# SHI-Labs/Self-Similarity-Grouping

Measured on AMD Instinct MI355X. Metric: images/s embed + s/iter for NxN rerank+DBSCAN, N=16k, 1/2/4/8 GPU, higher is better.
Workload: dtype f32 (embed: split-half operands hi+lo on fp16 MFMA, fp32 accumulate, 6e-8 max error vs the fp32 reference features) / exact int64 via int8 MFMA digits + f64 + f16 (distance, re-rank: half semantics, bit-exact)

## Files before the change

self-similarity-grouping_amd/csrc/conv.hip:

```cpp
#include "ssg_common.h"
#include <cstdlib>
#include <type_traits>

namespace ssg {

typedef float v16f __attribute__((ext_vector_type(16)));
typedef unsigned int v4u __attribute__((ext_vector_type(4)));
typedef _Float16 v8h __attribute__((ext_vector_type(8)));

__device__ __forceinline__ unsigned pack_h2(_Float16 a, _Float16 b) {
  return (unsigned)__builtin_bit_cast(unsigned short, a) | ((unsigned)__builtin_bit_cast(unsigned short, b) << 16);
}
__device__ __forceinline__ float unpack_lo(unsigned u) { return (float)__builtin_bit_cast(_Float16, (unsigned short)(u & 0xffffu)); }
__device__ __forceinline__ float unpack_hi(unsigned u) { return (float)__builtin_bit_cast(_Float16, (unsigned short)(u >> 16)); }
__device__ __forceinline__ void split_encode4(const float4 v, uint2& hi, uint2& lo) {
  const _Float16 h0 = (_Float16)v.x, h1 = (_Float16)v.y, h2 = (_Float16)v.z, h3 = (_Float16)v.w;
  hi = make_uint2(pack_h2(h0, h1), pack_h2(h2, h3));
  lo = make_uint2(pack_h2((_Float16)(v.x - (float)h0), (_Float16)(v.y - (float)h1)), pack_h2((_Float16)(v.z - (float)h2), (_Float16)(v.w - (float)h3)));
}
__device__ __forceinline__ bool split_hi_nonfinite(const uint2 hi) {
  const unsigned a = hi.x & 0x7fff7fffu, b = hi.y & 0x7fff7fffu;
  return (a & 0xffffu) >= 0x7c00u || (a >> 16) >= 0x7c00u || (b & 0xffffu) >= 0x7c00u || (b >> 16) >= 0x7c00u;
}
__device__ __forceinline__ float4 split_decode4(const uint2 hi, const uint2 lo) {
// ... 776 lines not shown
            const unsigned a0 = rr[it][0], a1 = rr[it][1], a2 = rr[it][2], a3 = rr[it][3];
            if (n + 1 < NP) rr[it] = __builtin_amdgcn_raw_buffer_load_b128(res_rsrc, poff(n + 1, it), 0, SSG_DMA_RES_AUX);
            const unsigned g0 = lane_xor1(odd ? a0 : a2), g1 = lane_xor1(odd ? a1 : a3);
            const float4 r4 = split_decode4(make_uint2(odd ? g0 : a0, odd ? g1 : a1), make_uint2(odd ? a2 : g0, odd ? a3 : g1));
            v.x += r4.x; v.y += r4.y; v.z += r4.z; v.w += r4.w;
          }
          v.x = v.x > 0.f ? v.x : 0.f; v.y = v.y > 0.f ? v.y : 0.f; v.z = v.z > 0.f ? v.z : 0.f; v.w = v.w > 0.f ? v.w : 0.f;
          uint2 hp, lp;
          split_encode4(v, hp, lp);
          ovf |= ((hp.x & 0x7c007c00u) + 0x04000400u) | ((hp.y & 0x7c007c00u) + 0x04000400u);
          const unsigned rx = lane_xor1(odd ? hp.x : lp.x), ry = lane_xor1(odd ? hp.y : lp.y);
          const v4u stv = {odd ? rx : hp.x, odd ? ry : hp.y, odd ? lp.x : rx, odd ? lp.y : ry};
          __builtin_amdgcn_raw_buffer_store_b128(stv, out_rsrc, poff(n, it), 0, RES ? SSG_DMA_OUT_AUX_RES : SSG_DMA_OUT_AUX);
        }
        __builtin_amdgcn_fence(__ATOMIC_ACQ_REL, "wavefront");
        if (n % MT == MT - 1) { bias = bias_n; cs = cs_n; }
      }
    };
    if (resp) run(std::true_type{}); else run(std::false_type{});
    if ((ovf & 0x80008000u) && p.overflow) *p.overflow = 1;
    SSG_DMA_STAMP(4)
    return;
  }
#pragma unroll
  for (int i = 0; i < MT; i++) {
    const int mbase = tm * BM + wm * WM + i * 32;
#pragma unroll
    for (int j = 0; j < NT; j++) {
      const int col = tn * BN + wn * WN + j * 32 + chunk * 4;
      const float4 bias = *reinterpret_cast<const float4*>(p.bias + col);
      const float4 cs = p.cscale ? *reinterpret_cast<const float4*>(p.cscale + col) : make_float4(1.f, 1.f, 1.f, 1.f);
      float4 rr[ITS];
      if (resp) {
#pragma unroll
        for (int it = 0; it < ITS; it++) {
          const int m = mbase + it * RPI + prow;
          rr[it] = *reinterpret_cast<const float4*>(resp + (int64_t)(m < p.M ? m : 0) * p.Cout + col);
        }
      }
#pragma unroll
      for (int q = 0; q < 4; q++)
        *reinterpret_cast<float4*>(patch + l32 * EP + 8 * q + 4 * h) = make_float4(acc[i][j][4 * q], acc[i][j][4 * q + 1], acc[i][j][4 * q + 2], acc[i][j][4 * q + 3]);
      __builtin_amdgcn_fence(__ATOMIC_ACQ_REL, "wavefront");
#pragma unroll
      for (int it = 0; it < ITS; it++) {
        const int m = mbase + it * RPI + prow;
        float4 v = *reinterpret_cast<const float4*>(patch + (it * RPI + prow) * EP + chunk * 4);
        v.x = v.x * cs.x + bias.x; v.y = v.y * cs.y + bias.y; v.z = v.z * cs.z + bias.z; v.w = v.w * cs.w + bias.w;
        if (resp) {
          float4 r4 = rr[it];
          if (p.res_split) {
            const unsigned s0 = odd ? __float_as_uint(r4.x) : __float_as_uint(r4.z), s1 = odd ? __float_as_uint(r4.y) : __float_as_uint(r4.w);
            const unsigned g0 = lane_xor1(s0), g1 = lane_xor1(s1);
            r4 = odd ? split_decode4(make_uint2(g0, g1), make_uint2(__float_as_uint(r4.z), __float_as_uint(r4.w)))
                     : split_decode4(make_uint2(__float_as_uint(r4.x), __float_as_uint(r4.y)), make_uint2(g0, g1));
          }
          v.x += r4.x; v.y += r4.y; v.z += r4.z; v.w += r4.w;
        }
        if (p.relu) { v.x = v.x > 0.f ? v.x : 0.f; v.y = v.y > 0.f ? v.y : 0.f; v.z = v.z > 0.f ? v.z : 0.f; v.w = v.w > 0.f ? v.w : 0.f; }
        if (p.out_split) {
          uint2 hp, lp;
          split_encode4(v, hp, lp);
          if (p.overflow && split_hi_nonfinite(hp)) *p.overflow = 1;
          const uint2 send = odd ? hp : lp;
          const uint2 recv = make_uint2(lane_xor1(send.x), lane_xor1(send.y));
          const uint4 stv = odd ? make_uint4(recv.x, recv.y, lp.x, lp.y) : make_uint4(hp.x, hp.y, recv.x, recv.y);
          if (m < p.M) *reinterpret_cast<uint4*>(outp + (int64_t)m * p.Cout + col) = stv;
        } else if (m < p.M) *reinterpret_cast<float4*>(outp + (int64_t)m * p.Cout + col) = v;
      }
      __builtin_amdgcn_fence(__ATOMIC_ACQ_REL, "wavefront");
    }
  }
}

__global__ void nchw_to_nhwc4_kernel(const float* __restrict__ in, float* __restrict__ out, int B, int H, int W, int flip) {
  const int64_t total = (int64_t)B * H * W;
  for (int64_t x = (int64_t)blockIdx.x * blockDim.x + threadIdx.x; x < total; x += (int64_t)gridDim.x * blockDim.x) {
    const int w = (int)(x % W); const int64_t t = x / W; const int hh = (int)(t % H); const int b = (int)(t / H);
    const int ws = flip ? (W - 1 - w) : w;
    const int64_t plane = (int64_t)H * W, base = (int64_t)b * 3 * plane + (int64_t)hh * W + ws;
    reinterpret_cast<float4*>(out)[x] = make_float4(in[base], in[base + plane], in[base + 2 * plane], 0.f);
  }
}

__global__ void nchw_to_nhwc4_h4l4_kernel(const float* __restrict__ in, float* __restrict__ out, int B, int H, int W, int flip) {
  const int64_t total = (int64_t)B * H * W;
  for (int64_t x = (int64_t)blockIdx.x * blockDim.x + threadIdx.x; x < total; x += (int64_t)gridDim.x * blockDim.x) {
    const int w = (int)(x % W); const int64_t t = x / W; const int hh = (int)(t % H); const int b = (int)(t / H);
    const int ws = flip ? (W - 1 - w) : w;
    const int64_t plane = (int64_t)H * W, base = (int64_t)b * 3 * plane + (int64_t)hh * W + ws;
    uint2 hi, lo;
    split_encode4(make_float4(in[base], in[base + plane], in[base + 2 * plane], 0.f), hi, lo);
    reinterpret_cast<uint4*>(out)[x] = make_uint4(hi.x, hi.y, lo.x, lo.y);
  }
}

__global__ void maxpool3x3s2_kernel(const float* __restrict__ in, float* __restrict__ out, int B, int H, int W, int C, int OH, int OW) {
  const int C4 = C / 4;
  const int64_t total = (int64_t)B * OH * OW * C4;
  for (int64_t x = (int64_t)blockIdx.x * blockDim.x + threadIdx.x; x < total; x += (int64_t)gridDim.x * blockDim.x) {
    const int c4 = (int)(x % C4); int64_t t = x / C4;
    const int ow = (int)(t % OW); t /= OW; const int oh = (int)(t % OH); const int b = (int)(t / OH);
    float4 m = make_float4(-INFINITY, -INFINITY, -INFINITY, -INFINITY);
    for (int r = 0; r < 3; r++) {
      const int ih = oh * 2 - 1 + r; if (ih < 0 || ih >= H) continue;
      for (int s = 0; s < 3; s++) {
        const int iw = ow * 2 - 1 + s; if (iw < 0 || iw >= W) continue;
        const float4 v = reinterpret_cast<const float4*>(in + ((int64_t)(b * H + ih) * W + iw) * C)[c4];
        m.x = fmaxf(m.x, v.x); m.y = fmaxf(m.y, v.y); m.z = fmaxf(m.z, v.z); m.w = fmaxf(m.w, v.w);
      }
    }
    reinterpret_cast<float4*>(out)[x] = m;
  }
}

__global__ void gap_stripes_kernel(const float* __restrict__ in, float* __restrict__ out, int B, int H, int W, int C, int S) {
  const int nsets = S > 1 ? S + 1 : 1;
  const int64_t total = (int64_t)nsets * B * C;
  for (int64_t x = (int64_t)blockIdx.x * blockDim.x + threadIdx.x; x < total; x += (int64_t)gridDim.x * blockDim.x) {
    const int c = (int)(x % C); int64_t t = x / C; const int b = (int)(t % B); const int s = (int)(t / B);
    int h0 = 0, h1 = H;
    if (s > 0) { const int hs = H / S; h0 = hs * (s - 1); h1 = hs * s; }
    float acc = 0.f;
    for (int hh = h0; hh < h1; hh++)
      for (int w = 0; w < W; w++) acc += in[((int64_t)(b * H + hh) * W + w) * C + c];
    out[x] = acc / (float)((h1 - h0) * W);
  }
}

__device__ __forceinline__ void h8l8_load8(const float* g, float4& a, float4& b) {
  const uint4 hi = *reinterpret_cast<const uint4*>(g), lo = *reinterpret_cast<const uint4*>(g + 4);
  a = split_decode4(make_uint2(hi.x, hi.y), make_uint2(lo.x, lo.y));
  b = split_decode4(make_uint2(hi.z, hi.w), make_uint2(lo.z, lo.w));
}
__device__ __forceinline__ void h8l8_store8(float* g, const float4 a, const float4 b) {
  uint2 ha, la, hb, lb;
  split_encode4(a, ha, la); split_encode4(b, hb, lb);
  *reinterpret_cast<uint4*>(g) = make_uint4(ha.x, ha.y, hb.x, hb.y);
  *reinterpret_cast<uint4*>(g + 4) = make_uint4(la.x, la.y, lb.x, lb.y);
}

__global__ void maxpool3x3s2_h8l8_kernel(const float* __restrict__ in, float* __restrict__ out, int B, int H, int W, int C, int OH, int OW) {
  const int C8 = C / 8;
  const int64_t total = (int64_t)B * OH * OW * C8;
  for (int64_t x = (int64_t)blockIdx.x * blockDim.x + threadIdx.x; x < total; x += (int64_t)gridDim.x * blockDim.x) {
    const int c8 = (int)(x % C8); int64_t t = x / C8;
    const int ow = (int)(t % OW); t /= OW; const int oh = (int)(t % OH); const int b = (int)(t / OH);
    float4 m0 = make_float4(-INFINITY, -INFINITY, -INFINITY, -INFINITY), m1 = m0;
    for (int r = 0; r < 3; r++) {
      const int ih = oh * 2 - 1 + r; if (ih < 0 || ih >= H) continue;
      for (int s = 0; s < 3; s++) {
        const int iw = ow * 2 - 1 + s; if (iw < 0 || iw >= W) continue;
        float4 a, c;
        h8l8_load8(in + ((int64_t)(b * H + ih) * W + iw) * C + c8 * 8, a, c);
        m0.x = fmaxf(m0.x, a.x); m0.y = fmaxf(m0.y, a.y); m0.z = fmaxf(m0.z, a.z); m0.w = fmaxf(m0.w, a.w);
        m1.x = fmaxf(m1.x, c.x); m1.y = fmaxf(m1.y, c.y); m1.z = fmaxf(m1.z, c.z); m1.w = fmaxf(m1.w, c.w);
      }
    }
    h8l8_store8(out + x * 8, m0, m1);
  }
}

__global__ void gap_stripes_h8l8_kernel(const float* __restrict__ in, float* __restrict__ out, int B, int H, int W, int C, int S) {
  const int nsets = S > 1 ? S + 1 : 1;
  const int64_t total = (int64_t)nsets * B * C;
  const unsigned short* hp = reinterpret_cast<const unsigned short*>(in);
  for (int64_t x = (int64_t)blockIdx.x * blockDim.x + threadIdx.x; x < total; x += (int64_t)gridDim.x * blockDim.x) {
    const int c = (int)(x % C); int64_t t = x / C; const int b = (int)(t % B); const int s = (int)(t / B);
    int h0 = 0, h1 = H;
    if (s > 0) { const int hs = H / S; h0 = hs * (s - 1); h1 = hs * s; }
    float acc = 0.f;
    for (int hh = h0; hh < h1; hh++)
      for (int w = 0; w < W; w++) {
        const int64_t e = (((int64_t)(b * H + hh) * W + w) * C + (c & ~7)) * 2 + (c & 7);
        acc += (float)__builtin_bit_cast(_Float16, hp[e]) + (float)__builtin_bit_cast(_Float16, hp[e + 8]);
      }
    out[x] = acc / (float)((h1 - h0) * W);
  }
}

__global__ void h8l8_encode_kernel(const float* __restrict__ in, float* __restrict__ out, int64_t ngroups, float scale) {
  for (int64_t x = (int64_t)blockIdx.x * blockDim.x + threadIdx.x; x < ngroups; x += (int64_t)gridDim.x * blockDim.x) {
    float4 a = reinterpret_cast<const float4*>(in)[2 * x], b = reinterpret_cast<const float4*>(in)[2 * x + 1];
    a.x *= scale; a.y *= scale; a.z *= scale; a.w *= scale; b.x *= scale; b.y *= scale; b.z *= scale; b.w *= scale;
    h8l8_store8(out + x * 8, a, b);
  }
}
__global__ void h8l8_decode_kernel(const float* __restrict__ in, float* __restrict__ out, int64_t ngroups, float scale) {
  for (int64_t x = (int64_t)blockIdx.x * blockDim.x + threadIdx.x; x < ngroups; x += (int64_t)gridDim.x * blockDim.x) {
    float4 a, b;
    h8l8_load8(in + x * 8, a, b);
    a.x *= scale; a.y *= scale; a.z *= scale; a.w *= scale; b.x *= scale; b.y *= scale; b.z *= scale; b.w *= scale;
    reinterpret_cast<float4*>(out)[2 * x] = a; reinterpret_cast<float4*>(out)[2 * x + 1] = b;
  }
}

__global__ __launch_bounds__(256) void flip_sum_l2norm_kernel(const float* __restrict__ a, const float* __restrict__ b, float* __restrict__ out,
                                                              int rows, int C) {
  const int row = (int)((blockIdx.x * blockDim.x + threadIdx.x) >> 6);
  if (row >= rows) return;
  const int lane = lane_id();
  const float* pa = a + (int64_t)row * C; const float* pb = b + (int64_t)row * C;
  float ss = 0.f;
  for (int c = lane; c < C; c += 64) { const float s = pa[c] + pb[c]; ss += s * s; }
  for (int sh = 1; sh < 64; sh <<= 1) ss += __shfl_xor(ss, sh, 64);
  const float nrm = sqrtf(ss);
  for (int c = lane; c < C; c += 64) out[(int64_t)row * C + c] = (pa[c] + pb[c]) / nrm;
}

}

using namespace ssg;

template <int BM, int BN, int WM, int WN, bool CIN4, int CBK, bool SPLIT>
static int launch_conv_bk(const ConvParams& p, hipStream_t stream) {
  const size_t lds = 2 * (size_t)(BM + BN) * (CBK + 4) * sizeof(float);
  const int tiles = ((p.M + BM - 1) / BM) * (p.Cout / BN);
  static bool attr_set = false;
  if (lds > 64 * 1024 && !attr_set) {
    int rc = ssg_check_hip(hipFuncSetAttribute((const void*)conv_igemm_kernel<BM, BN, WM, WN, CIN4, CBK, SPLIT>, hipFuncAttributeMaxDynamicSharedMemorySize, (int)lds),
                           "hipFuncSetAttribute(conv)");
    if (rc) return rc;
    attr_set = true;
  }
  hipLaunchKernelGGL((conv_igemm_kernel<BM, BN, WM, WN, CIN4, CBK, SPLIT>), dim3(tiles), dim3((BM / WM) * (BN / WN) * 64), lds, stream, p);
  return ssg_check_hip(hipGetLastError(), "conv_igemm_kernel");
}
template <int BM, int BN, int WM, int WN, bool CIN4>
static int launch_conv(const ConvParams& p, hipStream_t stream, bool split = false) {
  static int bk16_max = -1;
  if (bk16_max < 0) { const char* e = getenv("SSG_CONV_BK16_MAXK"); bk16_max = e ? atoi(e) : 0x7fffffff; }
  if (split) {
    if constexpr (CIN4) return launch_conv_bk<BM, BN, WM, WN, true, 16, true>(p, stream);
    else {
      static int sbk16 = -1;
      if (sbk16 < 0) { const char* e = getenv("SSG_SPLIT_BK16"); sbk16 = e ? atoi(e) : 0; }
      if (!p.in2 && p.Kpad <= sbk16) return launch_conv_bk<BM, BN, WM, WN, false, 16, true>(p, stream);
      if constexpr (BM == 128 && BN == 128) {
        static int dma = -1;
        if (dma < 0) { const char* e = getenv("SSG_CONV_DMA"); dma = e ? atoi(e) : 3; }
        if ((dma & 2) && p.epi == 0 && !p.in2) {
          const int tiles = ((p.M + 127) / 128) * (p.Cout / 128);
          hipLaunchKernelGGL(conv_dma_kernel<128>, dim3(tiles), dim3(256), 0, stream, p);
          return ssg_check_hip(hipGetLastError(), "conv_dma_kernel<128>");
        }
      }
      return launch_conv_bk<BM, BN, WM, WN, false, 32, true>(p, stream);
    }
  }
  if (!p.in2 && p.Kpad <= bk16_max) return launch_conv_bk<BM, BN, WM, WN, CIN4, 16, false>(p, stream);
  return launch_conv_bk<BM, BN, WM, WN, CIN4, 32, false>(p, stream);
}

static bool conv_prefers_wide(const ConvParams& p, bool split) {
  static int mintiles = -1;
  if (mintiles < 0) { const char* e = getenv("SSG_SPLIT_WIDE_MINTILES"); mintiles = e ? atoi(e) : 256; }
  if (!split || mintiles <= 0 || (p.Cout % 256) || p.Kpad < 128) return false;
  return ((p.M + 127) / 128) * (p.Cout / 256) >= mintiles;
}

static int launch_conv_wide(const ConvParams& p, hipStream_t stream) {
  static int dma = -1;
  if (dma < 0) { const char* e = getenv("SSG_CONV_DMA"); dma = e ? atoi(e) : 3; }
  if ((dma & 1) && (p.epi == 0 || p.epi == 3) && (int64_t)p.Cout * p.Kpad * 4 < 0x7fffffffLL) {
    static int tall = -1;
    if (tall < 0) { const char* e = getenv("SSG_CONV_TALL_MINTILES"); tall = e ? atoi(e) : 200; }
    const int tiles_tall = ((p.M + 255) / 256) * (p.Cout / 256);
    static int tall_dual = -1;
    if (tall_dual < 0) { const char* e = getenv("SSG_CONV_TALL_DUAL"); tall_dual = e ? atoi(e) : 0; }
    if (tall > 0 && p.products == 3 && p.epi == 0 && p.in2 && tall_dual && tiles_tall >= tall) {
      hipLaunchKernelGGL((conv_dma_kernel<256, false, 256, true, 4>), dim3(tiles_tall), dim3(1024), 0, stream, p);
      return ssg_check_hip(hipGetLastError(), "conv_dma_kernel<256x256, dual>");
    }
    static int tall_res = -1;
    if (tall_res < 0) { const char* e = getenv("SSG_CONV_TALL_RES"); tall_res = e ? atoi(e) : 0; }
    if (tall > 0 && p.products == 3 && p.epi == 0 && (!p.res || tall_res) && !p.in2 && tiles_tall >= tall) {
      static int tall_ns = -1;
      if (tall_ns < 0) { const char* e = getenv("SSG_CONV_TALL_STAGES"); tall_ns = e ? atoi(e) : 4; }
      static int tall_wm = -1;
      if (tall_wm < 0) { const char* e = getenv("SSG_CONV_TALL_WM"); tall_wm = e ? atoi(e) : 64; }
      if (tall_wm == 128) hipLaunchKernelGGL((conv_dma_kernel<256, false, 256, false, 4, 128, false>), dim3(tiles_tall), dim3(512), 0, stream, p);
      else if (tall_wm == 129) hipLaunchKernelGGL((conv_dma_kernel<256, false, 256, false, 4, 128, true>), dim3(tiles_tall), dim3(512), 0, stream, p);
      else if (tall_ns == 4) hipLaunchKernelGGL((conv_dma_kernel<256, false, 256, false, 4>), dim3(tiles_tall), dim3(1024), 0, stream, p);
      else hipLaunchKernelGGL((conv_dma_kernel<256, false, 256, false>), dim3(tiles_tall), dim3(1024), 0, stream, p);
      return ssg_check_hip(hipGetLastError(), "conv_dma_kernel<256x256>");
    }
    const int tiles = ((p.M + 127) / 128) * (p.Cout / 256);
    if (p.products == 1) hipLaunchKernelGGL((conv_dma_kernel<256, true>), dim3(tiles), dim3(512), 0, stream, p);
    else if (p.in2) hipLaunchKernelGGL((conv_dma_kernel<256, false, 128, true>), dim3(tiles), dim3(512), 0, stream, p);
    else hipLaunchKernelGGL(conv_dma_kernel<256>, dim3(tiles), dim3(512), 0, stream, p);
    return ssg_check_hip(hipGetLastError(), "conv_dma_kernel");
  }
  return launch_conv_bk<128, 256, 64, 64, false, 32, true>(p, stream);
}

static bool conv_prefers_bn64(const ConvParams& p, bool split) {
  static int maxtiles = -1;
  if (maxtiles < 0) { const char* e = getenv("SSG_SPLIT_BN64_MAXTILES"); maxtiles = e ? atoi(e) : 300; }
  if (!split) return false;
  const int tiles = ((p.M + 127) / 128) * (p.Cout / 128);
  return tiles < maxtiles;
}

extern "C" int ssg_conv2d_nhwc_x(const void* in, const void* w, const float* bias, const void* res, void* out, int B, int H, int W,
                                 int Cin, int Cout, int KH, int KW, int stride, int pad, int relu, int flags, float acc_scale, const float* ch_scale,
                                 int32_t* overflow, hipStream_t stream) {
  ConvParams p;
  p.cscale = ch_scale; p.overflow = overflow;
  p.in = (const float*)in; p.w = (const float*)w; p.bias = bias; p.res = (const float*)res; p.out = (float*)out;
  p.B = B; p.H = H; p.W = W; p.Cin = Cin; p.Cout = Cout; p.KH = KH; p.KW = KW; p.stride = stride; p.pad = pad; p.relu = relu;
  p.OH = (H + 2 * pad - KH) / stride + 1; p.OW = (W + 2 * pad - KW) / stride + 1;
  const int64_t M = (int64_t)B * p.OH * p.OW;
  const bool split = (flags & 1) != 0;
  if (B <= 0 || M <= 0 || M > 0x7fffffff || (Cout % 64) || !((Cin % 32) == 0 || Cin == 4) || stride < 1) {
    ssg_set_error("ssg_conv2d_nhwc: unsupported shape B=%d H=%d W=%d Cin=%d Cout=%d k=%dx%d s=%d p=%d flags=%d", B, H, W, Cin, Cout, KH, KW, stride, pad, flags);
    return SSG_ERR_INVALID;
  }
  p.M = (int)M;
  const int64_t in_bytes = (int64_t)B * H * W * Cin * 4;
  if (in_bytes > 0x7fffffffLL) { ssg_set_error("ssg_conv2d_nhwc: input tensor of %lld bytes exceeds the 2 GiB buffer-resource range of this kernel; use a smaller batch", (long long)in_bytes); return SSG_ERR_INVALID; }
  p.in_bytes = (unsigned)in_bytes;
  p.in2 = nullptr; p.H2 = p.W2 = p.Cin2 = 0; p.stride2 = 1; p.in2_bytes = 0; p.rowterm = nullptr; p.epi = 0; p.tilemin = nullptr; p.tmin_ld = 0;
  p.out_split = (flags & 2) ? 1 : 0; p.res_split = p.out_split; p.acc_scale = acc_scale;
  static int variant = -1;
  if (variant < 0) { const char* e = getenv("SSG_CONV_VARIANT"); variant = e ? atoi(e) : 0; }
  p.variant = variant;
  const bool cin4 = (Cin == 4);
  p.Kpad = cin4 ? 32 * ((KH * KW + 7) / 8) : KH * KW * Cin;
  p.nk1 = p.Kpad / 16;
  if (cin4) return (Cout % 128 == 0) ? launch_conv<128, 128, 64, 64, true>(p, stream, split) : launch_conv<128, 64, 64, 32, true>(p, stream, split);
  if (conv_prefers_wide(p, split)) return launch_conv_wide(p, stream);
  return (Cout % 128 == 0 && !conv_prefers_bn64(p, split)) ? launch_conv<128, 128, 64, 64, false>(p, stream, split) : launch_conv<128, 64, 64, 32, false>(p, stream, split);
}

extern "C" int ssg_conv2d_nhwc_f32(const float* in, const float* w, const float* bias, const float* res, float* out, int B, int H, int W,
                                   int Cin, int Cout, int KH, int KW, int stride, int pad, int relu, hipStream_t stream) {
  return ssg_conv2d_nhwc_x(in, w, bias, res, out, B, H, W, Cin, Cout, KH, KW, stride, pad, relu, 0, 1.f, nullptr, nullptr, stream);
}

extern "C" int ssg_conv1x1_dual_nhwc_x(const void* in, const void* in2, const void* w, const float* bias, void* out, int B, int H, int W,
                                       int Cin, int H2, int W2, int Cin2, int stride2, int Cout, int relu, int flags, float acc_scale, const float* ch_scale,
                                       int32_t* overflow, hipStream_t stream) {
  ConvParams p;
  p.cscale = ch_scale; p.overflow = overflow;
  p.in = (const float*)in; p.w = (const float*)w; p.bias = bias; p.res = nullptr; p.out = (float*)out;
  p.B = B; p.H = H; p.W = W; p.Cin = Cin; p.Cout = Cout; p.KH = 1; p.KW = 1; p.stride = 1; p.pad = 0; p.relu = relu;
  p.OH = H; p.OW = W;
  const int64_t M = (int64_t)B * H * W;
  const int64_t in_bytes = M * Cin * 4, in2_bytes = (int64_t)B * H2 * W2 * Cin2 * 4;
  if (B <= 0 || M > 0x7fffffff || (Cout % 64) || (Cin % 32) || (Cin2 % 32) || stride2 < 1 || (H - 1) * stride2 >= H2 || (W - 1) * stride2 >= W2 ||
      in_bytes > 0x7fffffffLL || in2_bytes > 0x7fffffffLL) {
    ssg_set_error("ssg_conv1x1_dual_nhwc: unsupported shape B=%d H=%d W=%d Cin=%d H2=%d W2=%d Cin2=%d s2=%d Cout=%d", B, H, W, Cin, H2, W2, Cin2, stride2, Cout);
    return SSG_ERR_INVALID;
  }
  p.M = (int)M; p.in_bytes = (unsigned)in_bytes;
  p.in2 = (const float*)in2; p.H2 = H2; p.W2 = W2; p.Cin2 = Cin2; p.stride2 = stride2; p.in2_bytes = (unsigned)in2_bytes;
  p.Kpad = Cin + Cin2; p.nk1 = Cin / 32; p.variant = 0; p.rowterm = nullptr; p.epi = 0; p.tilemin = nullptr; p.tmin_ld = 0;
  p.out_split = (flags & 2) ? 1 : 0; p.res_split = p.out_split; p.acc_scale = acc_scale;
  const bool split = (flags & 1) != 0;
  if (conv_prefers_wide(p, split)) return launch_conv_wide(p, stream);
  return (Cout % 128 == 0 && !conv_prefers_bn64(p, split)) ? launch_conv<128, 128, 64, 64, false>(p, stream, split) : launch_conv<128, 64, 64, 32, false>(p, stream, split);
}

extern "C" int ssg_conv1x1_dual_nhwc_f32(const float* in, const float* in2, const float* w, const float* bias, float* out, int B, int H, int W,
                                         int Cin, int H2, int W2, int Cin2, int stride2, int Cout, int relu, hipStream_t stream) {
  return ssg_conv1x1_dual_nhwc_x(in, in2, w, bias, out, B, H, W, Cin, H2, W2, Cin2, stride2, Cout, relu, 0, 1.f, nullptr, nullptr, stream);
}

namespace ssg {
__global__ __launch_bounds__(256) void row_sqnorm_kernel(const float* __restrict__ x, int rows, int d, float scale, float* __restrict__ out) {
  const int row = (int)((blockIdx.x * blockDim.x + threadIdx.x) >> 6);
  if (row >= rows) return;
  const int lane = lane_id();
  float s = 0.f;
  const float* xr = x + (int64_t)row * d;
  for (int c0 = lane; c0 < d; c0 += 512) {
    float v[8];
#pragma unroll
    for (int u = 0; u < 8; u++) v[u] = xr[min(c0 + 64 * u, d - 1)];
#pragma unroll
    for (int u = 0; u < 8; u++) if (c0 + 64 * u < d) s += v[u] * v[u];
  }
  for (int sh = 1; sh < 64; sh <<= 1) s += __shfl_xor(s, sh, 64);
  if (lane == 0) out[row] = s * scale;
}
}

extern "C" int ssg_pairwise_sqdist_f32(const float* x, const float* y, int m, int n, int d, int self_form, float* ws, float* out, hipStream_t stream) {
  if (m <= 0 || n <= 0 || (d % 32) || (n % 64) || (int64_t)m * d * 4 > 0x7fffffffLL) {
    ssg_set_error("ssg_pairwise_sqdist_f32: need d %% 32 == 0, n %% 64 == 0 and x < 2 GiB (m=%d n=%d d=%d)", m, n, d);
    return SSG_ERR_INVALID;
  }
  float* rowterm = ws; float* colterm = ws + m;
  hipLaunchKernelGGL(row_sqnorm_kernel, dim3((m + 3) / 4), dim3(256), 0, stream, x, m, d, self_form ? 2.f : 1.f, rowterm);
  hipLaunchKernelGGL(row_sqnorm_kernel, dim3((n + 3) / 4), dim3(256), 0, stream, y, n, d, self_form ? 0.f : 1.f, colterm);
  ConvParams p;
  p.in = x; p.w = y; p.bias = colterm; p.res = nullptr; p.out = out;
  p.B = m; p.H = 1; p.W = 1; p.Cin = d; p.Cout = n; p.KH = 1; p.KW = 1; p.stride = 1; p.pad = 0; p.relu = 0; p.OH = 1; p.OW = 1;
  p.M = m; p.Kpad = d; p.nk1 = d / 16; p.variant = 0; p.in_bytes = (unsigned)((int64_t)m * d * 4);
  p.in2 = nullptr; p.H2 = p.W2 = p.Cin2 = 0; p.stride2 = 1; p.in2_bytes = 0; p.rowterm = rowterm; p.epi = 1; p.tilemin = nullptr; p.tmin_ld = 0; p.out_split = p.res_split = 0; p.acc_scale = 1.f;
  return (n % 128 == 0) ? launch_conv<128, 128, 64, 64, false>(p, stream) : launch_conv<128, 64, 64, 32, false>(p, stream);
}

extern "C" int ssg_cosine_dist_f32(const float* x, const float* y, int m, int n, int d, const float* zeros, float* out, hipStream_t stream) {
  if (m <= 0 || n <= 0 || (d % 32) || (n % 64) || (int64_t)m * d * 4 > 0x7fffffffLL) {
    ssg_set_error("ssg_cosine_dist_f32: need d %% 32 == 0, n %% 64 == 0 and x < 2 GiB (m=%d n=%d d=%d)", m, n, d);
    return SSG_ERR_INVALID;
  }
  ConvParams p;
  p.in = x; p.w = y; p.bias = zeros; p.res = nullptr; p.out = out;
  p.B = m; p.H = 1; p.W = 1; p.Cin = d; p.Cout = n; p.KH = 1; p.KW = 1; p.stride = 1; p.pad = 0; p.relu = 0; p.OH = 1; p.OW = 1;
  p.M = m; p.Kpad = d; p.nk1 = d / 16; p.variant = 0; p.in_bytes = (unsigned)((int64_t)m * d * 4);
  p.in2 = nullptr; p.H2 = p.W2 = p.Cin2 = 0; p.stride2 = 1; p.in2_bytes = 0; p.rowterm = nullptr; p.epi = 2; p.tilemin = nullptr; p.tmin_ld = 0; p.out_split = p.res_split = 0; p.acc_scale = 1.f;
  return (n % 128 == 0) ? launch_conv<128, 128, 64, 64, false>(p, stream) : launch_conv<128, 64, 64, 32, false>(p, stream);
}


extern "C" int ssg_nchw_to_nhwc4(const float* in, float* out, int B, int H, int W, int flip, hipStream_t stream) {
  if (B <= 0 || H <= 0 || W <= 0) { ssg_set_error("ssg_nchw_to_nhwc4: empty"); return SSG_ERR_INVALID; }
  hipLaunchKernelGGL(nchw_to_nhwc4_kernel, dim3(4096), dim3(256), 0, stream, in, out, B, H, W, flip);
  SSG_LAUNCH_CHECK("nchw_to_nhwc4_kernel");
  return SSG_OK;
}

extern "C" int ssg_nchw_to_nhwc4_h4l4(const float* in, void* out, int B, int H, int W, int flip, hipStream_t stream) {
  if (B <= 0 || H <= 0 || W <= 0) { ssg_set_error("ssg_nchw_to_nhwc4_h4l4: empty"); return SSG_ERR_INVALID; }
  hipLaunchKernelGGL(nchw_to_nhwc4_h4l4_kernel, dim3(4096), dim3(256), 0, stream, in, (float*)out, B, H, W, flip);
  SSG_LAUNCH_CHECK("nchw_to_nhwc4_h4l4_kernel");
  return SSG_OK;
}

extern "C" int ssg_maxpool3x3s2_nhwc(const float* in, float* out, int B, int H, int W, int C, hipStream_t stream) {
  if (B <= 0 || (C & 3)) { ssg_set_error("ssg_maxpool3x3s2_nhwc: C %% 4 != 0"); return SSG_ERR_INVALID; }
  const int OH = (H + 2 - 3) / 2 + 1, OW = (W + 2 - 3) / 2 + 1;
  hipLaunchKernelGGL(maxpool3x3s2_kernel, dim3(8192), dim3(256), 0, stream, in, out, B, H, W, C, OH, OW);
  SSG_LAUNCH_CHECK("maxpool3x3s2_kernel");
  return SSG_OK;
}

extern "C" int ssg_maxpool3x3s2_h8l8(const void* in, void* out, int B, int H, int W, int C, hipStream_t stream) {
  if (B <= 0 || (C & 7)) { ssg_set_error("ssg_maxpool3x3s2_h8l8: C %% 8 != 0"); return SSG_ERR_INVALID; }
  const int OH = (H + 2 - 3) / 2 + 1, OW = (W + 2 - 3) / 2 + 1;
  hipLaunchKernelGGL(maxpool3x3s2_h8l8_kernel, dim3(8192), dim3(256), 0, stream, (const float*)in, (float*)out, B, H, W, C, OH, OW);
  SSG_LAUNCH_CHECK("maxpool3x3s2_h8l8_kernel");
  return SSG_OK;
}

extern "C" int ssg_gap_stripes_h8l8(const void* in, float* out, int B, int H, int W, int C, int num_split, hipStream_t stream) {
  if (B <= 0 || H <= 0 || W <= 0 || C <= 0 || (C & 7) || num_split > H) { ssg_set_error("ssg_gap_stripes_h8l8: bad shape"); return SSG_ERR_INVALID; }
  hipLaunchKernelGGL(gap_stripes_h8l8_kernel, dim3(2048), dim3(256), 0, stream, (const float*)in, out, B, H, W, C, num_split);
  SSG_LAUNCH_CHECK("gap_stripes_h8l8_kernel");
  return SSG_OK;
}

extern "C" int ssg_h8l8_encode(const float* in, void* out, int64_t n, float scale, hipStream_t stream) {
  if (n <= 0 || (n & 7)) { ssg_set_error("ssg_h8l8_encode: n must be a positive multiple of 8"); return SSG_ERR_INVALID; }
  hipLaunchKernelGGL(h8l8_encode_kernel, dim3(4096), dim3(256), 0, stream, in, (float*)out, n / 8, scale);
  SSG_LAUNCH_CHECK("h8l8_encode_kernel");
  return SSG_OK;
}

extern "C" int ssg_h8l8_decode(const void* in, float* out, int64_t n, float scale, hipStream_t stream) {
  if (n <= 0 || (n & 7)) { ssg_set_error("ssg_h8l8_decode: n must be a positive multiple of 8"); return SSG_ERR_INVALID; }
  hipLaunchKernelGGL(h8l8_decode_kernel, dim3(4096), dim3(256), 0, stream, (const float*)in, out, n / 8, scale);
  SSG_LAUNCH_CHECK("h8l8_decode_kernel");
  return SSG_OK;
}

extern "C" int ssg_gap_stripes(const float* in, float* out, int B, int H, int W, int C, int num_split, hipStream_t stream) {
  if (B <= 0 || H <= 0 || W <= 0 || C <= 0 || num_split > H) { ssg_set_error("ssg_gap_stripes: bad shape"); return SSG_ERR_INVALID; }
  hipLaunchKernelGGL(gap_stripes_kernel, dim3(2048), dim3(256), 0, stream, in, out, B, H, W, C, num_split);
  SSG_LAUNCH_CHECK("gap_stripes_kernel");
  return SSG_OK;
}

extern "C" int ssg_flip_sum_l2norm(const float* a, const float* b, float* out, int rows, int C, hipStream_t stream) {
  if (rows <= 0 || C <= 0) { ssg_set_error("ssg_flip_sum_l2norm: empty"); return SSG_ERR_INVALID; }
  hipLaunchKernelGGL(flip_sum_l2norm_kernel, dim3((rows + 3) / 4), dim3(256), 0, stream, a, b, out, rows, C);
  SSG_LAUNCH_CHECK("flip_sum_l2norm_kernel");
  return SSG_OK;
}
```

Baseline: 27630.

## Add specialized 256x256 3x3 conv kernel with resident input patch tiles

Adds a dedicated kernel for 3x3 stride-1 pad-1 convolutions where the spatial plane divides 256 and the split-half output path applies. It loads a 256-pixel input chunk once into LDS and reuses it across all nine taps through shifted row addressing and a validity mask, while a four-stage ring streams the weights. It uses 1024-thread blocks with 256x256 tiles and an in-LDS epilogue. The aim is to cut redundant im2col-style input reloads and raise MFMA reuse, at the cost of one block per CU and a narrow shape gate.

```diff
diff --git a/self-similarity-grouping_amd/csrc/conv.hip b/self-similarity-grouping_amd/csrc/conv.hip
--- a/self-similarity-grouping_amd/csrc/conv.hip
+++ b/self-similarity-grouping_amd/csrc/conv.hip
@@ -1102,6 +1102,8 @@
   return tiles < maxtiles;
 }
 
+#include "conv3x3_res.hip"
+
 extern "C" int ssg_conv2d_nhwc_x(const void* in, const void* w, const float* bias, const void* res, void* out, int B, int H, int W,
                                  int Cin, int Cout, int KH, int KW, int stride, int pad, int relu, int flags, float acc_scale, const float* ch_scale,
                                  int32_t* overflow, hipStream_t stream) {
@@ -1129,6 +1131,7 @@
   p.Kpad = cin4 ? 32 * ((KH * KW + 7) / 8) : KH * KW * Cin;
   p.nk1 = p.Kpad / 16;
   if (cin4) return (Cout % 128 == 0) ? launch_conv<128, 128, 64, 64, true>(p, stream, split) : launch_conv<128, 64, 64, 32, true>(p, stream, split);
+  if (conv3x3_res_takes(p, split)) return launch_conv3x3_res(p, stream);
   if (conv_prefers_wide(p, split)) return launch_conv_wide(p, stream);
   return (Cout % 128 == 0 && !conv_prefers_bn64(p, split)) ? launch_conv<128, 128, 64, 64, false>(p, stream, split) : launch_conv<128, 64, 64, 32, false>(p, stream, split);
 }
diff --git a/self-similarity-grouping_amd/csrc/conv3x3_res.hip b/self-similarity-grouping_amd/csrc/conv3x3_res.hip
--- /dev/null
+++ b/self-similarity-grouping_amd/csrc/conv3x3_res.hip
@@ -0,0 +1,209 @@
+#include "ssg_common.h"
+
+namespace ssg {
+
+template <int MT, int NT, int BM, int BN, int WM, int WN>
+__device__ __forceinline__ void conv3x3_res_epilogue(const ConvParams& p, v16f (&acc)[MT][NT], float* patch, const int tm, const int tn, const int wm, const int wn,
+                                                     const int lane) {
+  constexpr int EP = 36, CPR = 8, RPI = 8, ITS = 4, NP = MT * NT;
+  const int l32 = lane & 31, h = lane >> 5, chunk = lane % CPR, prow = lane / CPR, odd = lane & 1;
+  unsigned ovf = 0u;
+  const unsigned tbytes = (unsigned)((int64_t)p.M * p.Cout * 4), rowb = (unsigned)p.Cout * 4u;
+  const __amdgpu_buffer_rsrc_t out_rsrc = __builtin_amdgcn_make_buffer_rsrc(p.out, 0, tbytes, 0x00020000);
+  const unsigned lane_off = (unsigned)prow * rowb + (unsigned)chunk * 16u;
+  const unsigned ubase = (unsigned)(tm * BM + wm * WM) * rowb + (unsigned)(tn * BN + wn * WN) * 4u;
+  auto poff = [&](const int n, const int it) { return ubase + (unsigned)((n % MT) * 32 + it * RPI) * rowb + (unsigned)(n / MT) * 128u + lane_off; };
+  v4f bias = *reinterpret_cast<const v4f*>(p.bias + tn * BN + wn * WN + chunk * 4), cs = *reinterpret_cast<const v4f*>(p.cscale + tn * BN + wn * WN + chunk * 4);
+  v4f bias_n = bias, cs_n = cs;
+#pragma unroll
+  for (int n = 0; n < NP; n++) {
+    const int j = n / MT, i = n % MT;
+    if (n % MT == MT - 1 && j + 1 < NT) {
+      bias_n = *reinterpret_cast<const v4f*>(p.bias + tn * BN + wn * WN + (j + 1) * 32 + chunk * 4);
+      cs_n = *reinterpret_cast<const v4f*>(p.cscale + tn * BN + wn * WN + (j + 1) * 32 + chunk * 4);
+    }
+#pragma unroll
+    for (int q = 0; q < 4; q++)
+      *reinterpret_cast<float4*>(patch + l32 * EP + 8 * q + 4 * h) = make_float4(acc[i][j][4 * q], acc[i][j][4 * q + 1], acc[i][j][4 * q + 2], acc[i][j][4 * q + 3]);
+    __builtin_amdgcn_fence(__ATOMIC_ACQ_REL, "wavefront");
+#pragma unroll
+    for (int it = 0; it < ITS; it++) {
+      float4 v = *reinterpret_cast<const float4*>(patch + (it * RPI + prow) * EP + chunk * 4);
+      v.x = v.x * cs[0] + bias[0]; v.y = v.y * cs[1] + bias[1]; v.z = v.z * cs[2] + bias[2]; v.w = v.w * cs[3] + bias[3];
+      v.x = v.x > 0.f ? v.x : 0.f; v.y = v.y > 0.f ? v.y : 0.f; v.z = v.z > 0.f ? v.z : 0.f; v.w = v.w > 0.f ? v.w : 0.f;
+      uint2 hp, lp;
+      split_encode4(v, hp, lp);
+      ovf |= ((hp.x & 0x7c007c00u) + 0x04000400u) | ((hp.y & 0x7c007c00u) + 0x04000400u);
+      const unsigned rx = lane_xor1(odd ? hp.x : lp.x), ry = lane_xor1(odd ? hp.y : lp.y);
+      const v4u stv = {odd ? rx : hp.x, odd ? ry : hp.y, odd ? lp.x : rx, odd ? lp.y : ry};
+      __builtin_amdgcn_raw_buffer_store_b128(stv, out_rsrc, poff(n, it), 0, SSG_DMA_OUT_AUX);
+    }
+    __builtin_amdgcn_fence(__ATOMIC_ACQ_REL, "wavefront");
+    if (n % MT == MT - 1) { bias = bias_n; cs = cs_n; }
+  }
+  if ((ovf & 0x80008000u) && p.overflow) *p.overflow = 1;
+}
+
+__global__ __launch_bounds__(1024, 1) void conv3x3_res_kernel(ConvParams p) {
+  constexpr int BM = 256, BN = 256, WM = 64, WN = 64, MT = 2, NT = 2, WCOLS = BN / WN, NS = 4;
+  constexpr int WST = BN * 64;
+  constexpr int PXB = BM * 128;
+  __shared__ __attribute__((aligned(1024))) unsigned char ws0[WST];
+  __shared__ __attribute__((aligned(1024))) unsigned char ws1[WST];
+  __shared__ __attribute__((aligned(1024))) unsigned char ws2[WST];
+  __shared__ __attribute__((aligned(1024))) unsigned char ws3[WST];
+  __shared__ __attribute__((aligned(1024))) unsigned char px0[PXB + 256];
+  __shared__ __attribute__((aligned(1024))) unsigned char px1[PXB + 256];
+  const int tiles_n = p.Cout / BN, tiles_m = (p.M + BM - 1) / BM;
+  const int tile = conv_xcd_remap((int)blockIdx.x, tiles_m * tiles_n);
+  const int tm = tile / tiles_n, tn = tile % tiles_n;
+  const int tid = (int)threadIdx.x, lane = tid & 63, wave = __builtin_amdgcn_readfirstlane(tid >> 6);
+  SSG_DMA_STAMP(0)
+  const int wm = wave / WCOLS, wn = wave % WCOLS, l32 = lane & 31, h = lane >> 5;
+  if (tid < 16) {
+    *reinterpret_cast<uint4*>(px0 + PXB + tid * 16) = make_uint4(0u, 0u, 0u, 0u);
+    *reinterpret_cast<uint4*>(px1 + PXB + tid * 16) = make_uint4(0u, 0u, 0u, 0u);
+  }
+
+  const __amdgpu_buffer_rsrc_t in_rsrc = __builtin_amdgcn_make_buffer_rsrc(const_cast<float*>(p.in), 0, p.in_bytes, 0x00020000);
+  const __amdgpu_buffer_rsrc_t w_rsrc = __builtin_amdgcn_make_buffer_rsrc(const_cast<float*>(p.w), 0, (unsigned)((int64_t)p.Cout * p.Kpad * 4), 0x00020000);
+  unsigned po0, po1;
+  {
+    const int prow = wave * 16 + (lane >> 3), ps = lane & 7;
+    const int m0 = tm * BM + prow, m1 = m0 + 8;
+    po0 = m0 < p.M ? (unsigned)m0 * (unsigned)p.Cin * 4u + (unsigned)((ps ^ ((prow >> 1) & 7)) << 4) : 0x80000000u;
+    po1 = m1 < p.M ? (unsigned)m1 * (unsigned)p.Cin * 4u + (unsigned)((ps ^ (((prow + 8) >> 1) & 7)) << 4) : 0x80000000u;
+  }
+  const int drow = lane >> 2, pc = lane & 3;
+  const unsigned wo0 = (unsigned)(((tn * BN + wave * 16 + drow) * p.Kpad + ((pc ^ ((drow >> 2) & 3)) * 4)) * 4);
+  const int nk = p.Kpad / 16, nch = p.Cin / 32;
+  int wt = 0;
+#define C3_WS(S_) ((S_) % 4 == 0 ? ws0 : (S_) % 4 == 1 ? ws1 : (S_) % 4 == 2 ? ws2 : ws3)
+#define C3_DMA_W(WS_)                                                                                                            \
+  { __builtin_amdgcn_raw_ptr_buffer_load_lds(w_rsrc, SSG_LDSP(WS_ + wave * 1024), 16, wo0 + (unsigned)(wt * 64), 0, 0, 0);        \
+    wt = wt < nk - 1 ? wt + 1 : wt; }
+#define C3_DMA_P(PX_, CH_)                                                                                                       \
+  { __builtin_amdgcn_raw_ptr_buffer_load_lds(in_rsrc, SSG_LDSP(PX_ + wave * 2048), 16, po0 + (unsigned)((CH_) * 128), 0, 0, 0);   \
+    __builtin_amdgcn_raw_ptr_buffer_load_lds(in_rsrc, SSG_LDSP(PX_ + wave * 2048 + 1024), 16, po1 + (unsigned)((CH_) * 128), 0, 0, 0); }
+
+  const int g = (l32 >> 2) & 3;
+  const int offh = ((2 * h) ^ g) * 16, offl = ((2 * h + 1) ^ g) * 16;
+  const int brow = (wn * WN + l32) * 64;
+  const int row0 = wm * WM + l32;
+  unsigned vmask = 0u;
+  {
+    const int hw = p.H * p.W;
+#pragma unroll
+    for (int i = 0; i < MT; i++) {
+      const int pix = (row0 + i * 32) % hw, oh = pix / p.W, ow = pix - oh * p.W;
+#pragma unroll
+      for (int dr = 0; dr < 3; dr++)
+#pragma unroll
+        for (int ds = 0; ds < 3; ds++)
+          if ((unsigned)(oh + dr - 1) < (unsigned)p.H && (unsigned)(ow + ds - 1) < (unsigned)p.W) vmask |= 1u << (9 * i + 3 * dr + ds);
+    }
+  }
+
+  v16f acc[MT][NT];
+#pragma unroll
+  for (int i = 0; i < MT; i++)
+#pragma unroll
+    for (int j = 0; j < NT; j++)
+#pragma unroll
+      for (int r = 0; r < 16; r++) acc[i][j][r] = 0.f;
+
+  v8h fah[MT], fal[MT], fbh[NT], fbl[NT];
+  int pa0 = 0, pa1 = 0;
+#define C3_G1 { _Pragma("unroll") for (int i = 0; i < MT; i++) _Pragma("unroll") for (int j = 0; j < NT; j++)      \
+      acc[i][j] = __builtin_amdgcn_mfma_f32_32x32x16_f16(fbh[j], fal[i], acc[i][j], 0, 0, 0); }
+#define C3_G2 { _Pragma("unroll") for (int i = 0; i < MT; i++) _Pragma("unroll") for (int j = 0; j < NT; j++)      \
+      acc[i][j] = __builtin_amdgcn_mfma_f32_32x32x16_f16(fbl[j], fah[i], acc[i][j], 0, 0, 0); }
+#define C3_G3 { _Pragma("unroll") for (int i = 0; i < MT; i++) _Pragma("unroll") for (int j = 0; j < NT; j++)      \
+      acc[i][j] = __builtin_amdgcn_mfma_f32_32x32x16_f16(fbh[j], fah[i], acc[i][j], 0, 0, 0); }
+#define C3_STEP(S_, PX_, PXN_, CHN_)                                                                                             \
+  { constexpr int cs_ = (S_) % 18, tap_ = cs_ / 2, ks_ = cs_ & 1, dr_ = tap_ / 3, ds_ = tap_ % 3;                                 \
+    constexpr int vm_ = 2 + ((cs_ == 1 || cs_ == 2) ? 2 : 0);                                                                     \
+    if constexpr (ks_ == 0) {                                                                                                     \
+      int rl_ = row0; asm volatile("" : "+v"(rl_));    \
+      const int r_ = rl_ + (dr_ - 1) * p.W + (ds_ - 1);                                                                           \
+      const int v_ = r_ * 128 + (((2 * h) ^ ((r_ >> 1) & 7)) << 4);                                                                \
+      const int z_ = PXB + (v_ & 255);                                                                                            \
+      pa0 = (vmask >> (3 * dr_ + ds_)) & 1u ? v_ : z_;                                                                            \
+      pa1 = (vmask >> (9 + 3 * dr_ + ds_)) & 1u ? v_ + 32 * 128 : z_;                                                             \
+    }                                                                                                                             \
+    fah[0] = *reinterpret_cast<const v8h*>(PX_ + (pa0 ^ (ks_ * 64))); fal[0] = *reinterpret_cast<const v8h*>(PX_ + (pa0 ^ (ks_ * 64 + 16)));   \
+    fah[1] = *reinterpret_cast<const v8h*>(PX_ + (pa1 ^ (ks_ * 64))); fal[1] = *reinterpret_cast<const v8h*>(PX_ + (pa1 ^ (ks_ * 64 + 16)));   \
+    _Pragma("unroll") for (int j = 0; j < NT; j++) {                                                                              \
+      fbh[j] = *reinterpret_cast<const v8h*>(C3_WS(S_) + brow + j * 2048 + offh); fbl[j] = *reinterpret_cast<const v8h*>(C3_WS(S_) + brow + j * 2048 + offl); } \
+    C3_G1 C3_G2                                                                                                                   \
+    __builtin_amdgcn_sched_barrier(0);                                                                                            \
+    asm volatile("s_waitcnt vmcnt(%0) lgkmcnt(0)\n\ts_barrier" ::"n"(vm_) : "memory");                                            \
+    if constexpr (cs_ == 0) C3_DMA_P(PXN_, CHN_)                                                                                  \
+    C3_DMA_W(C3_WS(S_))                                                                                                           \
+    __builtin_amdgcn_sched_barrier(0);                                                                                            \
+    C3_G3 }
+#define C3_CHUNK(S0_, PX_, PXN_, CHN_)                                                                                           \
+  C3_STEP(S0_ + 0, PX_, PXN_, CHN_) C3_STEP(S0_ + 1, PX_, PXN_, CHN_) C3_STEP(S0_ + 2, PX_, PXN_, CHN_) C3_STEP(S0_ + 3, PX_, PXN_, CHN_)       \
+  C3_STEP(S0_ + 4, PX_, PXN_, CHN_) C3_STEP(S0_ + 5, PX_, PXN_, CHN_) C3_STEP(S0_ + 6, PX_, PXN_, CHN_) C3_STEP(S0_ + 7, PX_, PXN_, CHN_)       \
+  C3_STEP(S0_ + 8, PX_, PXN_, CHN_) C3_STEP(S0_ + 9, PX_, PXN_, CHN_) C3_STEP(S0_ + 10, PX_, PXN_, CHN_) C3_STEP(S0_ + 11, PX_, PXN_, CHN_)     \
+  C3_STEP(S0_ + 12, PX_, PXN_, CHN_) C3_STEP(S0_ + 13, PX_, PXN_, CHN_) C3_STEP(S0_ + 14, PX_, PXN_, CHN_) C3_STEP(S0_ + 15, PX_, PXN_, CHN_)   \
+  C3_STEP(S0_ + 16, PX_, PXN_, CHN_) C3_STEP(S0_ + 17, PX_, PXN_, CHN_)
+
+  C3_DMA_P(px0, 0)
+  C3_DMA_W(ws0)
+  C3_DMA_W(ws1)
+  C3_DMA_W(ws2)
+  C3_DMA_W(ws3)
+  asm volatile("s_waitcnt vmcnt(3) lgkmcnt(0)\n\ts_barrier" ::: "memory");
+  SSG_DMA_STAMP(1)
+  for (int c = 0; c < nch; c += 2) {
+    const int c2 = c + 2 < nch ? c + 2 : nch - 1;
+    C3_CHUNK(0, px0, px1, c + 1)
+    C3_CHUNK(18, px1, px0, c2)
+  }
+  SSG_DMA_STAMP(2)
+  __syncthreads();
+  SSG_DMA_STAMP(3)
+#undef C3_CHUNK
+#undef C3_STEP
+#undef C3_G1
+#undef C3_G2
+#undef C3_G3
+#undef C3_DMA_P
+#undef C3_DMA_W
+#undef C3_WS
+#pragma unroll
+  for (int i = 0; i < MT; i++)
+#pragma unroll
+    for (int j = 0; j < NT; j++)
+#pragma unroll
+      for (int r = 0; r < 16; r++) acc[i][j][r] *= p.acc_scale;
+  constexpr int PB = 32 * 36 * 4;
+  static_assert(7 * PB <= PXB + 256 && 2 * PB <= WST, "epilogue patches fit");
+  float* patch = reinterpret_cast<float*>(wave < 7 ? px0 + wave * PB : (wave < 14 ? px1 + (wave - 7) * PB : ws0 + (wave - 14) * PB));
+  conv3x3_res_epilogue<MT, NT, BM, BN, WM, WN>(p, acc, patch, tm, tn, wm, wn, lane);
+  SSG_DMA_STAMP(4)
+}
+
+static bool conv3x3_res_takes(const ConvParams& p, bool split) {
+  static int mode = -1, tall = -1, dma = -1;
+  if (mode < 0) { const char* e = getenv("SSG_CONV3_RES"); mode = e ? atoi(e) : 1; }
+  if (tall < 0) { const char* e = getenv("SSG_CONV_TALL_MINTILES"); tall = e ? atoi(e) : 200; }
+  if (dma < 0) { const char* e = getenv("SSG_CONV_DMA"); dma = e ? atoi(e) : 3; }
+  if (mode <= 0 || !split) return false;
+  const int hw = p.H * p.W;
+  const bool shape = p.KH == 3 && p.KW == 3 && p.stride == 1 && p.pad == 1 && hw > 0 && 256 % hw == 0 && p.Cin % 64 == 0 && p.Cout % 256 == 0;
+  const bool epi = p.epi == 0 && !p.in2 && !p.res && p.out_split && p.relu && p.cscale != nullptr && p.products == 3 && p.variant != 7 &&
+                   ((int64_t)p.M + 256) * p.Cout * 4 < (int64_t)0xffffffff && (int64_t)p.Cout * p.Kpad * 4 < 0x7fffffffLL;
+  if (!shape || !epi) return false;
+  if (mode >= 2) return true;
+  return (dma & 1) && tall > 0 && ((p.M + 255) / 256) * (p.Cout / 256) >= tall && conv_prefers_wide(p, split);
+}
+
+static int launch_conv3x3_res(const ConvParams& p, hipStream_t stream) {
+  const int tiles = ((p.M + 255) / 256) * (p.Cout / 256);
+  hipLaunchKernelGGL(conv3x3_res_kernel, dim3(tiles), dim3(1024), 0, stream, p);
+  return ssg_check_hip(hipGetLastError(), "conv3x3_res_kernel");
+}
+
+}
```

New measurement: 27970, median of 6. +1.2%, better.
